# SGI-2022/Latent-Diffusion-Models-for-Shape-SDFs

Measured on AMD Instinct MI355X. Metric: SDF queries/sec on 256^3 grid (+ DDPM sample steps/sec), higher is better.
Workload: dtype bf16; 1 GPU; config4: decode B=64 shapes on a 256^3 grid on 1 rank (the whole grid is the one slab: no gather); batch=64, grid=256, latent_dim=256, decoder=DeepSDF 8x512 skip@4, parallelism=zslab1

## Files before the change

### latent-diffusion-models-for-shape-sdfs_amd/csrc/decoder_fs.hip

```cpp
#include "decoder_common.h"

namespace ldm {
namespace {
using namespace dec;

constexpr int kFsD = 4;

constexpr int kFsStep = 2048;
constexpr int kFsAct = 33 * 4 * 1024;
constexpr int kFsRed = 4 * 4 * 64 * 4;
constexpr int kFsWl = 512 * 4;
#ifndef FS_STAMP
#define FS_STAMP 0
#endif
constexpr int kFsStamp = FS_STAMP ? 128 * 8 : 0;
#ifndef FS_ABL
#define FS_ABL 0
#endif
static_assert(FS_ABL == 0 || FS_STAMP, "ablations are diagnostic builds");
constexpr int kFsLds = kFsAct + kFsRed + kFsWl + kFsStamp;
static_assert(kFsLds <= 160 * 1024, "LDS");

__host__ __device__ constexpr int fs_nparts(int S) { return S == 256 ? 15 : 16; }
__host__ __device__ constexpr int fs_nsteps(int S) { return S == 256 ? 384 : 448; }

template <typename T>
__global__ void fs_aux_pack_kernel(const float* __restrict__ beta, const float* __restrict__ wxyz,
                                   int B, T* __restrict__ aux) {
    const int id = blockIdx.x * blockDim.x + threadIdx.x;
    if (id >= B * 4 * 4 * 2 * 64) return;
    const int lane = id & 63;
    const int i = (id >> 6) & 1;
    const int slot = (id >> 7) & 3;
    const int w = (id >> 9) & 3;
    const int b = id >> 11;
    const int li = slot >> 1;
    const int p = slot & 1;
    float v[8] = {0, 0, 0, 0, 0, 0, 0, 0};
    if (lane < 32) {
        const int f = 128 * w + 64 * p + 32 * i + lane;
        const float* wx = wxyz + ((size_t)li * kHidden + f) * 3;
        const float bb = beta[((size_t)b * 2 + li) * kHidden + f];
        const float hi = Elem<T>::round(bb);
        v[0] = wx[0]; v[1] = wx[1]; v[2] = wx[2];
        v[3] = wx[0]; v[4] = wx[1]; v[5] = wx[2];
        v[6] = hi;    v[7] = bb - hi;
    }
    T* o = aux + (size_t)id * 8;
#pragma unroll
    for (int e = 0; e < 8; ++e) o[e] = (T)v[e];
}

struct FArgs {
    const uint8_t* stream;
    const uint8_t* aux;
    const float* w_last;
    const float* xyz;
    float* out;
    float b_last;
    int npts, tiles_per_shape, n_tiles;
    int N, k0;
    float vs, origin;
    const int32_t* bricks;
    const int32_t* count;
    int nb, nbt;
    GridDiv gd;
};

enum FsEpi { FE_NONE = 0, FE_LATE = 1, FE_EARLY = 2, FE_FIN0 = 3, FE_FIN1 = 4 };

struct FSrc {
    bool shape;
    uint32_t off;
    bool none = false;
};

struct FCtx {
    int lane, wave, h;
    uint32_t voff;
    char* smem;
    __amdgpu_buffer_rsrc_t rw;
    __amdgpu_buffer_rsrc_t ra;
    uint32_t s_beg, s_end;
    uint32_t s_iss;
    uint32_t baux_w;
    uint32_t aux_w;
    uint32_t aux_next;
    u32x4 auxn[2];
    u32x4 ring[kFsD][2];
    u32x4 b[4];
    float part[4];
    const f32x4* wlp;
    f32x4 wl[2][4];
    float* out;
    int npts, prev_shape, prev_local;
    float b_last;
    unsigned long long* st;
    int st_i;
    bool st_on;
    const int32_t* bricks;
    int N, nb, nbt;
};

__device__ __forceinline__ void stamp(FCtx& c) {
    if (FS_STAMP) {
        if (c.st_on && c.lane == 0 && c.st_i < 128) c.st[c.st_i] = __builtin_readcyclecounter();
        ++c.st_i;
    }
}

__device__ __forceinline__ u32x4 bld(__amdgpu_buffer_rsrc_t r, uint32_t voff, uint32_t soff) {
    return __builtin_bit_cast(u32x4, __builtin_amdgcn_raw_buffer_load_b128(r, voff, soff, 0));
}

__device__ __forceinline__ void load_aux(FCtx& c, FSrc s) {
    if (s.none) return;
    const __amdgpu_buffer_rsrc_t r = s.shape ? c.ra : c.rw;
    c.auxn[0] = bld(r, c.voff, s.off);
    c.auxn[1] = bld(r, c.voff + 1024u, s.off);
}

__device__ __forceinline__ uint32_t opaque(uint32_t v) {
    asm volatile("" : "+v"(v));
    return v;
}

__device__ __forceinline__ int opaque_s(int v) {
    asm volatile("" : "+s"(v));
    return v;
}

__device__ __forceinline__ char* lds_at(const FCtx& c, uint32_t off) {
    return c.smem + (opaque(c.voff) + off);
}
__device__ __forceinline__ char* lds_base(const FCtx& c, uint32_t off) {
    return c.smem + opaque(opaque(c.voff) + off);
}
__device__ __forceinline__ u32x4* act_wb(const FCtx& c, int late) {
    return reinterpret_cast<u32x4*>(lds_base(c, (uint32_t)(late + 4 * c.wave) * 4096u));
}
__device__ __forceinline__ u32x4* act_w(const FCtx& c, int late) {
    return reinterpret_cast<u32x4*>(lds_at(c, (uint32_t)(late + 4 * c.wave) * 4096u));
}
__device__ __forceinline__ const f32x4* wl_at(const FCtx& c, int p, int i) {
    const uint32_t h = opaque(c.voff) >> 9;
    return reinterpret_cast<const f32x4*>(
        c.smem + kFsAct + kFsRed + (((c.wave * 2 + p) * 2 + i) * 2) * 64 + h * 64);
}

__device__ __forceinline__ float* red_w(const FCtx& c) {
    return reinterpret_cast<float*>(c.smem + kFsAct + c.wave * 4 * 64 * 4 + (opaque(c.voff) >> 2));
}

__device__ __forceinline__ void fs_bar() {
    if (FS_ABL & 4) return;
    asm volatile("s_waitcnt lgkmcnt(0)\n\ts_barrier" ::: "memory");
}

__device__ __forceinline__ void read_b(FCtx& c, int pos) {
    const u32x4* p = reinterpret_cast<const u32x4*>(lds_at(c, pos * 4096));
#pragma unroll
    for (int n = 0; n < 4; ++n) c.b[n] = p[n * 64];
}

__device__ __forceinline__ void issue(FCtx& c, int r) {
    const uint32_t so = c.s_iss + (uint32_t)(r >> 1) * 2u * kFsStep;
    const uint32_t vo = c.voff + (uint32_t)(r & 1) * kFsStep;
    if (FS_ABL & 1) return;
    c.ring[r][0] = bld(c.rw, vo, so);
    c.ring[r][1] = bld(c.rw, vo + 1024u, so);
}

__device__ __forceinline__ uint32_t next_iss(const FCtx& c) {
    const uint32_t n = c.s_iss + 4u * kFsStep;
    return n == c.s_end ? c.s_beg : n;
}
__device__ __forceinline__ void next_group(FCtx& c) { c.s_iss = next_iss(c); }

__device__ __forceinline__ float relu_f(float x) {
    return __builtin_bit_cast(float, max(__builtin_bit_cast(int, x), 0));
}

__device__ __forceinline__ float acc_read(float a) {
    asm volatile("" : "+a"(a));
    return a;
}

__device__ __forceinline__ void fin1_unit(FCtx& c, const f32x16 (&accY)[2][4], int u) {
    const int t = u >> 1, s = u & 1;
    const int i = t >> 2, n = t & 3;
    const f32x4* w = wl_at(c, 1, i);
    float part = c.part[n];
#pragma unroll
    for (int q = 2 * s; q < 2 * s + 2; ++q) {
        const f32x4 wv = w[q];
#pragma unroll
        for (int e = 0; e < 4; ++e)
            part = fmaf(relu_f(acc_read(accY[i][n][4 * q + e])), wv[e], part);
    }
    c.part[n] = part;
}

template <typename T>
__device__ __forceinline__ void mfma_pair(f32x16 (&acc)[2][4], const u32x4& a0, const u32x4& a1,
                                          const u32x4& b, int n) {
    acc[0][n] = Elem<T>::mfma(a0, b, acc[0][n]);
    acc[1][n] = Elem<T>::mfma(a1, b, acc[1][n]);
}

template <typename T>
__device__ __forceinline__ void window_step(FCtx& c, f32x16 (&acc)[2][4],
                                            const f32x16 (&accY)[2][4], const u32x4& a0,
                                            const u32x4& a1, const u32x4* nb, int k, int r,
                                            u32x4* wbase) {
    uint32_t nxt = 0;
    if (k < 14) {
        const int t = k >> 1, s = k & 1;
        const int i = t >> 2, nn = t & 3;
        u32x4 f;
#pragma unroll
        for (int n = 0; n < 4; ++n) {
            unsigned w;
            if (r == 3 && n == 1) nxt = next_iss(c);
            const float e0 = accY[i][nn][8 * s + 2 * n], e1 = accY[i][nn][8 * s + 2 * n + 1];
            if (n < 3)
                Elem<T>::template pair_cvt1<false>(acc[0][n], acc[1][n], a0, a1, c.b[n], e0, e1,
                                                   w);
            else
                Elem<T>::template pair_cvt1<true>(acc[0][n], acc[1][n], a0, a1, c.b[n], e0, e1,
                                                  w);
            f[n] = w;
            c.b[n] = nb[n * 64];
            __builtin_amdgcn_sched_barrier(0);
        }
        issue(c, r);
        wbase[((2 * i + s) * 4 + nn) * 64] = f;
        if (r == 3) c.s_iss = nxt;
    } else {
        u32x4 f[2];
        const f32x16& y = accY[1][3];
#pragma unroll
        for (int p = 0; p < 4; ++p) {
            unsigned w0, w1;
            if (p < 3)
                Elem<T>::template pair_cvt2<false>(acc[0][p], acc[1][p], a0, a1, c.b[p], y[4 * p],
                                                   y[4 * p + 1], y[4 * p + 2], y[4 * p + 3], w0,
                                                   w1);
            else
                Elem<T>::template pair_cvt2<true>(acc[0][p], acc[1][p], a0, a1, c.b[p], y[4 * p],
                                                  y[4 * p + 1], y[4 * p + 2], y[4 * p + 3], w0,
                                                  w1);
            f[p >> 1][2 * (p & 1)] = w0;
            f[p >> 1][2 * (p & 1) + 1] = w1;
            c.b[p] = nb[p * 64];
            if (p == 1) wbase[(2 * 4 + 3) * 64] = f[0];
            __builtin_amdgcn_sched_barrier(0);
        }
        issue(c, r);
        wbase[(3 * 4 + 3) * 64] = f[1];
    }
    __builtin_amdgcn_sched_barrier(0);
}

template <typename T, int P>
__device__ __forceinline__ void window_step_fin(FCtx& c, f32x16 (&acc)[2][4],
                                                const f32x16 (&accY)[2][4], const u32x4& a0,
                                                const u32x4& a1, const u32x4* nb, int k, int r) {
    const int t = k >> 1, s = k & 1;
    const int i = t >> 2, nn = t & 3;
    const f32x16& y = accY[1][3];
    uint32_t nxt = 0;
    if (k == 0) {
        c.wlp = wl_at(c, P, 0);
#pragma unroll
        for (int q = 0; q < 4; ++q) c.wl[0][q] = c.wlp[q];
    }
#pragma unroll
    for (int n = 0; n < 4; ++n) {
        if (k < 14) {
            const int e = 8 * s + 2 * n;
            const float e0 = accY[i][nn][e], e1 = accY[i][nn][e + 1];
            const float w0 = c.wl[i][e >> 2][e & 3], w1 = c.wl[i][e >> 2][(e & 3) + 1];
            const int x = 2 * (k - 8) + n;
            if (k >= 8 && n < 2)
                Elem<T>::pair_fin3(acc[0][n], acc[1][n], a0, a1, c.b[n], e0, e1, w0, w1,
                                   c.part[nn], y[x], c.wl[1][x >> 2][x & 3], c.part[3]);
            else if (n < 3)
                Elem<T>::template pair_fin<false>(acc[0][n], acc[1][n], a0, a1, c.b[n], e0, e1,
                                                  w0, w1, c.part[nn]);
            else
                Elem<T>::template pair_fin<true>(acc[0][n], acc[1][n], a0, a1, c.b[n], e0, e1,
                                                 w0, w1, c.part[nn]);
        } else if (n < 2) {
            const int x = 12 + 2 * n;
            Elem<T>::template pair_fin<false>(acc[0][n], acc[1][n], a0, a1, c.b[n], y[x],
                                              y[x + 1], c.wl[1][3][x & 3],
                                              c.wl[1][3][(x & 3) + 1],
                                              c.part[3]);
        } else {
            mfma_pair<T>(acc, a0, a1, c.b[n], n);
        }
        if (r == 3 && n == 2) nxt = next_iss(c);
        c.b[n] = nb[n * 64];
        if (k == 6) c.wl[1][n] = c.wlp[8 + n];
        if (k == 14 && n == 2) {
            if (P == 0) {
#pragma unroll
                for (int m = 0; m < 4; ++m) asm volatile("" : "+v"(c.part[m]));
            } else {
                float* rw = red_w(c);
#pragma unroll
                for (int m = 0; m < 4; ++m) {
                    rw[m * 64] = c.part[m];
                    c.part[m] = 0.f;
                }
            }
        }
        __builtin_amdgcn_sched_barrier(0);
    }
    issue(c, r);
    if (r == 3) c.s_iss = nxt;
    __builtin_amdgcn_sched_barrier(0);
}

__device__ __forceinline__ void fin_store(const FCtx& c, int shape, int local) {
    const int lane = (int)(opaque(c.voff) >> 4);
    if (local < 0 || lane >= 32) return;
    const float* rr = reinterpret_cast<const float*>(
        c.smem + kFsAct + c.wave * 64 * 4 + (opaque(c.voff) >> 2));
    float s = 0.f;
#pragma unroll
    for (int w = 0; w < 4; ++w) s += rr[w * 4 * 64] + rr[w * 4 * 64 + 32];
    const int pt = local * kTilePoints + 32 * c.wave + lane;
    if (pt < c.npts) {
        const __amdgpu_buffer_rsrc_t ro = __builtin_amdgcn_make_buffer_rsrc(
            (void*)(c.out + (size_t)shape * c.npts), (short)0, 0x7ffffff0, 0x00020000);
        __builtin_amdgcn_raw_buffer_store_b32(__builtin_bit_cast(uint32_t, tanhf(s + c.b_last)),
                                              ro, (uint32_t)pt * 4u, 0, 2 );
    }
}

__device__ __forceinline__ int list_at(const int32_t* list, int i) {
    typedef const __attribute__((address_space(4))) int32_t* const_i32;
    return ((const_i32)(uintptr_t)list)[i];
}

__device__ __forceinline__ void brick_origin(int gid, int nb_, int& shape, int& i0, int& j0,
                                             int& k0) {
    const int nb = opaque_s(nb_);
    const int nb2 = nb * nb, nb3 = nb2 * nb;
    shape = gid / nb3;
    const int id = gid - shape * nb3;
    const int bz = id / nb2, r = id - bz * nb2;
    const int by = r / nb;
    i0 = 8 * (r - by * nb);
    j0 = 8 * by;
    k0 = 8 * bz;
}

__device__ __forceinline__ void fin_store_bricks(const FCtx& c, int tile) {
    const int lane = (int)(opaque(c.voff) >> 4);
    if (tile < 0 || lane >= 32) return;
    const float* rr = reinterpret_cast<const float*>(
        c.smem + kFsAct + c.wave * 64 * 4 + (opaque(c.voff) >> 2));
    float s = 0.f;
#pragma unroll
    for (int w = 0; w < 4; ++w) s += rr[w * 4 * 64] + rr[w * 4 * 64 + 32];
    const int gid = list_at(c.bricks, tile >> 2);
    LDM_DASSERT(gid >= 0 && gid < c.nbt);
    int shape, i0, j0, k0;
    brick_origin(gid, c.nb, shape, i0, j0, k0);
    const int idx = 128 * (tile & 3) + 32 * c.wave + lane;
    const int i = i0 + (idx & 7), j = j0 + ((idx >> 3) & 7);
    const int k = k0 + 2 * (tile & 3) + (c.wave >> 1);
    const int N = c.N;
    if ((unsigned)gid < (unsigned)c.nbt && i < N && j < N && k < N) {
        const __amdgpu_buffer_rsrc_t ro = __builtin_amdgcn_make_buffer_rsrc(
            (void*)(c.out + ((size_t)shape * N + k) * N * N), (short)0, 0x7ffffff0, 0x00020000);
        __builtin_amdgcn_raw_buffer_store_b32(__builtin_bit_cast(uint32_t, tanhf(s + c.b_last)),
                                              ro, (uint32_t)(j * N + i) * 4u, 0, 2 );
    }
}

template <int MODE>
__device__ __forceinline__ void fin_store_mode(const FCtx& c) {
    if (MODE == kModeBricks) fin_store_bricks(c, c.prev_local);
    else fin_store(c, c.prev_shape, c.prev_local);
}

template <typename T, int EK, int K0, int BAR, bool WIN = false>
__device__ __forceinline__ void group4(FCtx& c, f32x16 (&acc)[2][4], const f32x16 (&accY)[2][4],
                                       int p0, const char* gb = nullptr, u32x4* wb = nullptr,
                                       uint32_t* go = nullptr) {
    static_assert(WIN || EK == FE_NONE, "windows run through steps16e");
    constexpr int BP = 1;
    const bool carry = go != nullptr;
    const char* gbase = WIN ? gb : carry ? c.smem + *go + 4096 : lds_base(c, (p0 + 1) * 4096);
#pragma unroll
    for (int r = 0; r < 4; ++r) {
        const bool last = carry && r == 3;
        uint32_t nxt = 0;
        if (last) {
            nxt = next_iss(c);
            *go = opaque(*go + 4u * 4096u);
        }
        const u32x4* nb =
            reinterpret_cast<const u32x4*>(last ? c.smem + *go : gbase + r * 4096);
        const u32x4 a0 = c.ring[r][0], a1 = c.ring[r][1];
        const int k = K0 + r;
        if (r == BAR) {
#pragma unroll
            for (int n = 0; n < BP; ++n) mfma_pair<T>(acc, a0, a1, c.b[n], n);
            for (int n = 0; n < BP; ++n) {
                __builtin_amdgcn_sched_group_barrier(0x008, 2, 0);
            }
            __builtin_amdgcn_sched_barrier(0);
            fs_bar();
            __builtin_amdgcn_sched_barrier(0);
#pragma unroll
            for (int n = 0; n < BP; ++n) c.b[n] = nb[n * 64];
#pragma unroll
            for (int n = BP; n < 4; ++n) {
                mfma_pair<T>(acc, a0, a1, c.b[n], n);
                c.b[n] = nb[n * 64];
            }
            issue(c, r);
            for (int n = 0; n < BP; ++n) __builtin_amdgcn_sched_group_barrier(0x100, 1, 0);
            for (int n = BP; n < 4; ++n) {
                __builtin_amdgcn_sched_group_barrier(0x008, 2, 0);
                __builtin_amdgcn_sched_group_barrier(0x100, 1, 0);
            }
        } else if ((EK == FE_LATE || EK == FE_EARLY) && k < 15 && !(FS_ABL & 2)) {
            window_step<T>(c, acc, accY, a0, a1, nb, k, r, wb);
            if (r == 3) return;
            continue;
        } else if ((EK == FE_FIN0 || EK == FE_FIN1) && k < 15 && !(FS_ABL & 2)) {
            window_step_fin<T, EK == FE_FIN1>(c, acc, accY, a0, a1, nb, k, r);
            if (r == 3) return;
            continue;
        } else {
#pragma unroll
            for (int n = 0; n < 4; ++n) {
                mfma_pair<T>(acc, a0, a1, c.b[n], n);
                c.b[n] = nb[n * 64];
            }
            issue(c, r);
            if (last) c.s_iss = nxt;
#pragma unroll
            for (int n = 0; n < 4; ++n) {
                __builtin_amdgcn_sched_group_barrier(0x008, 2, 0);
                if (last && n == 0) {
                    __builtin_amdgcn_sched_group_barrier(0x004, 3, 0);
                    __builtin_amdgcn_sched_group_barrier(0x002, 1, 0);
                }
                __builtin_amdgcn_sched_group_barrier(0x100, 1, 0);
            }
        }
        __builtin_amdgcn_sched_group_barrier(0x020, 2, 0);
        __builtin_amdgcn_sched_barrier(0);
    }
    if (!carry) next_group(c);
}

template <typename T, int EK, bool BAR>
__device__ __forceinline__ void steps16e(FCtx& c, f32x16 (&acc)[2][4],
                                         const f32x16 (&accY)[2][4], int p0) {
    const char* gb = lds_base(c, (p0 + 1) * 4096);
    u32x4* wb = EK == FE_LATE ? act_wb(c, 16) : EK == FE_EARLY ? act_wb(c, 0) : nullptr;
    group4<T, EK, 0, -1, true>(c, acc, accY, p0, gb, wb);
    group4<T, EK, 4, -1, true>(c, acc, accY, p0 + 4, gb + 4 * 4096, wb);
    group4<T, EK, 8, -1, true>(c, acc, accY, p0 + 8, gb + 8 * 4096, wb);
    group4<T, EK, 12, BAR ? 3 : -1, true>(c, acc, accY, p0 + 12, gb + 12 * 4096, wb);
}

template <typename T>
__device__ __forceinline__ void steps_plain(FCtx& c, f32x16 (&acc)[2][4],
                                            const f32x16 (&accY)[2][4], int pos0, int j0, int j1) {
    if (j0 >= j1) return;
    uint32_t go = opaque(opaque(c.voff) + (uint32_t)(pos0 + j0) * 4096u);
#pragma unroll 1
    for (int j = j0; j < j1; j += 4)
        group4<T, FE_NONE, 0, -1>(c, acc, accY, pos0 + j, nullptr, nullptr, &go);
}

template <typename T, int EK, bool E16, int MODE = kModeGrid>
__device__ __forceinline__ void run_part(FCtx& c, f32x16 (&acc)[2][4], const f32x16 (&accY)[2][4],
                                         int nk, bool mid, bool endbar, FSrc naux, int pos0,
                                         bool bar0) {
    const f32x16 zero = {};
    const u32x4 a0 = c.auxn[0], a1 = c.auxn[1];
    if (bar0) {
#pragma unroll
        for (int n = 0; n < 4; ++n) {
            acc[0][n] = Elem<T>::mfma(a0, c.b[n], zero);
            acc[1][n] = Elem<T>::mfma(a1, c.b[n], zero);
        }
        load_aux(c, naux);
        fs_bar();
        read_b(c, pos0);
    } else {
        const u32x4* p = reinterpret_cast<const u32x4*>(lds_at(c, pos0 * 4096));
#pragma unroll
        for (int n = 0; n < 4; ++n) {
            acc[0][n] = Elem<T>::mfma(a0, c.b[n], zero);
            acc[1][n] = Elem<T>::mfma(a1, c.b[n], zero);
            c.b[n] = p[n * 64];
        }
        load_aux(c, naux);
#pragma unroll
        for (int n = 0; n < 4; ++n) {
            __builtin_amdgcn_sched_group_barrier(0x008, 2, 0);
            __builtin_amdgcn_sched_group_barrier(0x100, 1, 0);
        }
        __builtin_amdgcn_sched_group_barrier(0x020, 2, 0);
        __builtin_amdgcn_sched_barrier(0);
    }
    if (EK == FE_NONE) {
#pragma unroll
        for (int i = 0; i < 2; ++i)
#pragma unroll
            for (int n = 0; n < 4; ++n) asm volatile("" ::"a"(accY[i][n]));
    }
    stamp(c);
    if (!E16 && EK != FE_NONE) {
        if (mid || (endbar && nk == 16)) steps16e<T, EK, true>(c, acc, accY, pos0);
        else steps16e<T, EK, false>(c, acc, accY, pos0);
        if (EK == FE_FIN1) {
            stamp(c);
            fin_store_mode<MODE>(c);
        }
        stamp(c);
        if (endbar && nk == 32) {
            steps_plain<T>(c, acc, accY, pos0, 16, 28);
            group4<T, FE_NONE, 0, 3>(c, acc, accY, pos0 + 28);
        } else {
            steps_plain<T>(c, acc, accY, pos0, 16, nk);
        }
    } else if (E16) {
        static_assert(!E16 || EK == FE_EARLY, "E16 parts convert part 0 of their own layer");
        steps_plain<T>(c, acc, accY, pos0, 0, 12);
        group4<T, FE_NONE, 0, 3>(c, acc, accY, pos0 + 12);
        stamp(c);
        if (endbar) steps16e<T, EK, true>(c, acc, accY, pos0 + 16);
        else steps16e<T, EK, false>(c, acc, accY, pos0 + 16);
    } else {
        steps_plain<T>(c, acc, accY, pos0, 0, nk < 16 ? nk : 16);
        stamp(c);
        steps_plain<T>(c, acc, accY, pos0, 16, nk);
    }
    stamp(c);
}

template <typename T>
__device__ __forceinline__ void acc_to_lds(FCtx& c, const f32x16 (&acc)[2][4]) {
    u32x4* p = act_w(c, 16);
#pragma unroll
    for (int i = 0; i < 2; ++i)
#pragma unroll
        for (int n = 0; n < 4; ++n) {
            u32x4 f0, f1;
            acc_to_frags<T>(acc[i][n], f0, f1);
            p[(2 * i * 4 + n) * 64] = f0;
            p[((2 * i + 1) * 4 + n) * 64] = f1;
        }
}

template <typename T, bool LATE>
__device__ __forceinline__ void layer0_part(FCtx& c, FSrc naux) {
    const u32x4 a[2] = {c.auxn[0], c.auxn[1]};
    u32x4* p = act_w(c, LATE ? 16 : 0);
    f32x16 t[2];
    t[0] = Elem<T>::mfma_v(a[0], c.b[0]);
#pragma unroll
    for (int q = 0; q < 8; ++q) {
        const int i = q & 1, n = q >> 1;
        if (q < 7) t[(q + 1) & 1] = Elem<T>::mfma_v(a[(q + 1) & 1], c.b[(q + 1) >> 1]);
        if (q == 0) {
            asm volatile("s_nop 10" : "+v"(t[0]));
            load_aux(c, naux);
            stamp(c);
        }
        __builtin_amdgcn_sched_barrier(0);
        u32x4 f0, f1;
        acc_to_frags<T>(t[q & 1], f0, f1);
        p[(2 * i * 4 + n) * 64] = f0;
        p[((2 * i + 1) * 4 + n) * 64] = f1;
        __builtin_amdgcn_sched_barrier(0);
    }
    stamp(c);
}

template <typename T, int S, int MODE>
__global__ __launch_bounds__(256, 1) void dec_fs_kernel(FArgs a) {
    __shared__ __attribute__((aligned(16))) char smem[kFsLds];
    FCtx c;
    c.lane = threadIdx.x & 63;
    c.wave = __builtin_amdgcn_readfirstlane(threadIdx.x >> 6);
    c.h = c.lane >> 5;
    c.voff = (uint32_t)c.lane * 16u;
    c.smem = smem;
    c.out = a.out;
    c.npts = a.npts;
    c.b_last = a.b_last;
    c.prev_shape = 0;
    c.prev_local = -1;
    c.st = reinterpret_cast<unsigned long long*>(smem + kFsAct + kFsRed + kFsWl);
    c.st_i = 0;
    c.st_on = false;
    float* wl = reinterpret_cast<float*>(smem + kFsAct + kFsRed);

    for (int i = threadIdx.x; i < 512; i += 256) wl[i] = a.w_last[i];
    __syncthreads();
    const int n_tiles = MODE == kModeBricks ? 4 * min(max(a.count[0], 0), a.nbt) : a.n_tiles;
    if (MODE == kModeBricks) {
        c.bricks = a.bricks;
        c.N = a.N;
        c.nb = a.nb;
        c.nbt = a.nbt;
    }
    if ((int)blockIdx.x >= n_tiles) return;

    constexpr int NST = fs_nsteps(S);
    constexpr int NP = fs_nparts(S);
    constexpr uint32_t kFlags = 0x00020000u;
    c.rw = __builtin_amdgcn_make_buffer_rsrc((void*)a.stream, (short)0, 0x7ffffff0, kFlags);
    c.ra = __builtin_amdgcn_make_buffer_rsrc((void*)a.aux, (short)0, 0x7ffffff0, kFlags);
    c.s_beg = (uint32_t)c.wave * NST * kFsStep;
    c.s_end = c.s_beg + NST * kFsStep;
    c.s_iss = c.s_beg;
    c.baux_w = (uint32_t)(4 * NST + c.wave * NP) * kFsStep;
    auto brick_of = [&](int tile) -> int {
        return min(max(list_at(a.bricks, tile >> 2), 0), a.nbt - 1);
    };
    auto shape_aux = [&](int tile) -> uint32_t {
        if (MODE == kModeBricks) {
            const int nb = opaque_s(a.nb);
            return ((uint32_t)(brick_of(tile) / (nb * nb * nb)) * 4u + (uint32_t)c.wave) * 4u *
                   kFsStep;
        }
        return ((uint32_t)(tile / a.tiles_per_shape) * 4u + (uint32_t)c.wave) * 4u * kFsStep;
    };
    auto bias = [&](int pi) -> FSrc { return FSrc{false, c.baux_w + (uint32_t)pi * kFsStep}; };
    auto shp = [&](int slot) -> FSrc { return FSrc{true, c.aux_w + (uint32_t)slot * kFsStep}; };
    c.aux_w = shape_aux(blockIdx.x);
#pragma unroll
    for (int r = 0; r < kFsD; ++r) issue(c, r);
    next_group(c);

    f32x16 accA[2][4], accB[2][4];
#pragma unroll
    for (int i = 0; i < 2; ++i)
#pragma unroll
        for (int n = 0; n < 4; ++n) accB[i][n] = f32x16{};
#pragma unroll
    for (int n = 0; n < 4; ++n) c.part[n] = 0.f;
#pragma unroll 1
    for (int tile = blockIdx.x; tile < n_tiles; tile += gridDim.x) {
        int shape, local, bi0 = 0, bj0 = 0, bk0 = 0;
        if (MODE == kModeBricks) {
            brick_origin(brick_of(tile), a.nb, shape, bi0, bj0, bk0);
            local = tile;
        } else {
            shape = tile / a.tiles_per_shape;
            local = tile - shape * a.tiles_per_shape;
        }
        {
            const int nt = tile + (int)gridDim.x;
            c.aux_next = nt < n_tiles ? shape_aux(nt) : c.aux_w;
        }
        c.st_on = FS_STAMP && c.wave == 0 && tile == (int)blockIdx.x + (int)gridDim.x;
        c.st_i = 0;
        stamp(c);
        load_aux(c, shp(0));
        const uint32_t lv = opaque(c.voff);
        const bool hi = lv >= 512u;
        const uint32_t p0 = (uint32_t)local * kTilePoints;
        uint32_t ti = 0, tj = 0, tk = 0;
        if (MODE == kModeGrid) {
            grid_first(p0, (uint32_t)a.N, a.gd, ti, tj, tk);
            tk += (uint32_t)a.k0;
        }
        const float* row = nullptr;
        if (MODE == kModePoints) {
            row = a.xyz + (size_t)shape * a.npts * 3;
            asm volatile("" : "+s"(row));
        }
#pragma unroll
        for (int n = 0; n < 4; ++n) {
            int pt = local * kTilePoints + 32 * n + (int)((lv >> 4) & 31u);
            if (pt >= a.npts) pt = a.npts - 1;
            float x, y, z;
            if (MODE == kModeBricks) {
                const int idx = 128 * (tile & 3) + 32 * n + (int)((lv >> 4) & 31u);
                const int m = a.N - 1;
                x = grid_axis(min(bi0 + (idx & 7), m), a.vs, a.origin);
                y = grid_axis(min(bj0 + ((idx >> 3) & 7), m), a.vs, a.origin);
                z = grid_axis(min(bk0 + (idx >> 6), m), a.vs, a.origin);
            } else if (MODE == kModePoints) {
                const float* qq = row + (size_t)pt * 3;
                x = qq[0];
                y = qq[1];
                z = qq[2];
            } else {
                const uint32_t off =
                    grid_tail_off(p0, 32u * n + ((lv >> 4) & 31u), (uint32_t)a.npts);
                uint32_t vi, vj, vk;
                grid_voxel(ti, tj, tk, off, (uint32_t)a.N, a.gd.m, vi, vj, vk);
                x = grid_axis((int)vi, a.vs, a.origin);
                y = grid_axis((int)vj, a.vs, a.origin);
                z = grid_axis((int)vk, a.vs, a.origin);
            }
            const float xh = Elem<T>::round(x), yh = Elem<T>::round(y), zh = Elem<T>::round(z);
            u32x4 f;
            f[0] = hi ? 0u : Elem<T>::pack(xh, yh);
            f[1] = hi ? 0u : Elem<T>::pack(zh, x - xh);
            f[2] = hi ? 0u : Elem<T>::pack(y - yh, z - zh);
            f[3] = hi ? 0u : Elem<T>::pack(1.f, 1.f);
            reinterpret_cast<u32x4*>(lds_at(c, 32u * 4096u))[n * 64] = f;
        }
        read_b(c, 32);

        layer0_part<T, false>(c, shp(1));
        layer0_part<T, true>(c, bias(2));

        int pi = 2;
        run_part<T, FE_FIN1, false, MODE>(c, accA, accB, 32, true, false, bias(pi + 1), 0, true);
        run_part<T, FE_EARLY, true>(c, accB, accA, 32, true, true, bias(pi + 2), 0, false);
        pi += 2;
        constexpr int L2P = S == 256 ? 3 : 4;
#pragma unroll 1
        for (int l = 2; l < L2P; ++l, pi += 2) {
            const FSrc nx = (S == 512 && l == 3) ? shp(2) : bias(pi + 2);
            run_part<T, FE_LATE, false>(c, accA, accB, 32, true, false, bias(pi + 1), 0,
                                                false);
            run_part<T, FE_EARLY, true>(c, accB, accA, 32, true, true, nx, 0, false);
        }
        if (S == 256) {
            run_part<T, FE_LATE, false>(c, accA, accB, 32, true, false, shp(2), 0,
                                                false);
            fs_bar();
            acc_to_lds<T>(c, accA);
            stamp(c);
            run_part<T, FE_NONE, false>(c, accA, accB, 16, false, false, shp(3), 16, true);
            run_part<T, FE_EARLY, false>(c, accB, accA, 16, false, true, bias(pi + 3),
                                                  16, false);
            pi += 3;
        } else {
            run_part<T, FE_LATE, false>(c, accA, accB, 32, true, false, shp(3), 0,
                                                false);
            run_part<T, FE_EARLY, true>(c, accB, accA, 32, true, true, bias(pi + 2), 0,
                                                 false);
            pi += 2;
        }
#pragma unroll 1
        for (int l = 5; l < 7; ++l, pi += 2) {
            run_part<T, FE_LATE, false>(c, accA, accB, 32, true, false, bias(pi + 1), 0,
                                                 false);
            run_part<T, FE_EARLY, true>(c, accB, accA, 32, true, true, bias(pi + 2), 0,
                                                 false);
        }
        run_part<T, FE_LATE, false>(c, accA, accB, 32, true, false, bias(pi + 1), 0,
                                             false);
        run_part<T, FE_FIN0, false>(c, accB, accA, 32, false, true, FSrc{true, 0, true},
                                             0, false);
        c.prev_shape = shape;
        c.prev_local = local;
        c.aux_w = c.aux_next;
    }
#pragma unroll
    for (int u = 0; u < 16; ++u) fin1_unit(c, accB, u);
    {
        float* rw = red_w(c);
#pragma unroll
        for (int n = 0; n < 4; ++n) rw[n * 64] = c.part[n];
    }
    fs_bar();
    fin_store_mode<MODE>(c);
    asm volatile("s_waitcnt vmcnt(0)" ::: "memory");
    if (FS_STAMP && c.wave == 0) {
        __builtin_amdgcn_s_waitcnt(0);
        for (int k = c.lane; k < 128; k += 64)
            reinterpret_cast<unsigned long long*>(a.out)[(size_t)blockIdx.x * 128 + k] = c.st[k];
    }
}

template <typename T, int S>
void launch_fs(const FArgs& a, bool points, hipStream_t s, int grid) {
    if (points)
        hipLaunchKernelGGL((dec_fs_kernel<T, S, kModePoints>), dim3(grid), dim3(256), 0, s, a);
    else
        hipLaunchKernelGGL((dec_fs_kernel<T, S, kModeGrid>), dim3(grid), dim3(256), 0, s, a);
}

template <typename T, int S>
void launch_fs_bricks(const FArgs& a, hipStream_t s, int grid) {
    hipLaunchKernelGGL((dec_fs_kernel<T, S, kModeBricks>), dim3(grid), dim3(256), 0, s, a);
}

}

size_t decoder_fs_aux_bytes(int B) { return (size_t)B * 4 * 4 * kFsStep; }

int decoder_fs_n_stages(int skip_width) { return fs_nsteps(skip_width == 253 ? 256 : 512); }

int decoder_fs_fwd(const ldm_decoder_t* w, const float* beta, const float* xyz, int B, int npts,
                   int N, int k0, float vs, float origin, float* out, void* ws, size_t ws_bytes,
                   hipStream_t s, int num_cus, const int32_t* bricks, const int32_t* count,
                   int n_bricks) {
    const int S = w->skip_width == 253 ? 256 : 512;
    LDM_REQUIRE(w->n_stages == fs_nsteps(S), LDM_EINVAL, "split layout: n_stages %d != %d",
                w->n_stages, fs_nsteps(S));
    LDM_REQUIRE(ws != nullptr && ws_bytes >= decoder_fs_aux_bytes(B) && LDM_ALIGNED(ws, 16),
                LDM_ENOSPC, "workspace too small: need %zu bytes, got %zu",
                decoder_fs_aux_bytes(B), ws_bytes);
    LDM_REQUIRE((size_t)B * 4 * 4 * kFsStep < 0x7ffffff0u, LDM_EINVAL,
                "split layout: %d shapes exceed the aux buffer range", B);
    {
        const int n = B * 4 * 4 * 2 * 64;
        if (w->dtype == LDM_BF16)
            hipLaunchKernelGGL(fs_aux_pack_kernel<__bf16>, dim3((n + 255) / 256), dim3(256), 0, s,
                               beta, w->wxyz, B, (__bf16*)ws);
        else
            hipLaunchKernelGGL(fs_aux_pack_kernel<_Float16>, dim3((n + 255) / 256), dim3(256), 0,
                               s, beta, w->wxyz, B, (_Float16*)ws);
        if (int e = launch_status("fs_aux_pack")) return e;
    }
    FArgs a;
    a.stream = (const uint8_t*)w->weights;
    a.aux = (const uint8_t*)ws;
    a.w_last = w->w_last;
    a.xyz = xyz;
    a.out = out;
    a.b_last = w->b_last;
    a.npts = npts;
    a.tiles_per_shape = (npts + kTilePoints - 1) / kTilePoints;
    a.n_tiles = B * a.tiles_per_shape;
    a.bricks = bricks;
    a.count = count;
    a.nb = (N + 7) / 8;
    a.nbt = n_bricks;
    const int mode = bricks ? kModeBricks : xyz ? kModePoints : kModeGrid;
    if (mode == kModeBricks) a.n_tiles = 4 * n_bricks;
    a.N = N;
    a.k0 = k0;
    a.vs = vs;
    a.origin = origin;
    a.gd = mode == kModeGrid ? grid_div(N) : GridDiv{0, 0, 0};
    const int grid = a.n_tiles < num_cus ? a.n_tiles : num_cus;
    if (mode != kModeBricks) {
        const bool points = mode == kModePoints;
        if (w->dtype == LDM_BF16) {
            if (S == 256) launch_fs<__bf16, 256>(a, points, s, grid);
            else launch_fs<__bf16, 512>(a, points, s, grid);
        } else {
            if (S == 256) launch_fs<_Float16, 256>(a, points, s, grid);
            else launch_fs<_Float16, 512>(a, points, s, grid);
        }
    } else if (w->dtype == LDM_BF16) {
        if (S == 256) launch_fs_bricks<__bf16, 256>(a, s, grid);
        else launch_fs_bricks<__bf16, 512>(a, s, grid);
    } else {
        if (S == 256) launch_fs_bricks<_Float16, 256>(a, s, grid);
        else launch_fs_bricks<_Float16, 512>(a, s, grid);
    }
    return launch_status("ldm_decoder_fwd(split)");
}

}
```

### latent-diffusion-models-for-shape-sdfs_amd/csrc/grid_index.h

```cpp
#pragma once
#include <stdint.h>

#if defined(__HIPCC__) || defined(__CUDACC__)
#define LDM_HD __host__ __device__ inline __attribute__((always_inline))
#else
#define LDM_HD inline
#endif

namespace ldm {
namespace dec {

struct GridDiv {
    uint32_t m, mw, sh;
};

inline GridDiv grid_div(int N) {
    GridDiv d;
    d.m = (uint32_t)(((1ull << 32) + (uint32_t)N - 1) / (uint32_t)N);
    uint32_t lg = 0;
    while ((1u << lg) < (uint32_t)N) ++lg;
    d.sh = 31 + lg;
    d.mw = (uint32_t)(((1ull << d.sh) + (uint32_t)N - 1) / (uint32_t)N);
    return d;
}

LDM_HD uint32_t grid_mulhi(uint32_t a, uint32_t b) {
    return (uint32_t)(((uint64_t)a * b) >> 32);
}

LDM_HD uint32_t grid_mul24(uint32_t a, uint32_t b) {
    return (a & 0xffffffu) * (b & 0xffffffu);
}

LDM_HD void grid_first(uint32_t p0, uint32_t N, GridDiv d, uint32_t& i, uint32_t& j,
                       uint32_t& k) {
    const uint32_t row = (uint32_t)(((uint64_t)p0 * d.mw) >> d.sh);
    i = p0 - row * N;
    k = grid_mulhi(row, d.m);
    j = row - k * N;
}

LDM_HD void grid_voxel(uint32_t i0, uint32_t j0, uint32_t k0, uint32_t off, uint32_t N,
                       uint32_t m, uint32_t& i, uint32_t& j, uint32_t& k) {
    const uint32_t x = i0 + off;
    const uint32_t cx = grid_mulhi(x, m);
    i = x - grid_mul24(cx, N);
    const uint32_t y = j0 + cx;
    const uint32_t cy = grid_mulhi(y, m);
    j = y - grid_mul24(cy, N);
    k = k0 + cy;
}

LDM_HD uint32_t grid_tail_off(uint32_t p0, uint32_t want, uint32_t npts) {
    const uint32_t last = npts - 1u - p0;
    return want < last ? want : last;
}

}
}
```

Baseline: 487.3 million queries/s.

## Interleave final tanh store into next layer's MFMA steps and simplify grid-row coordinates

Moves the final-layer reduction, tanh and output store of the previous tile out of its own serialized epilogue and splits it into pieces scheduled between the MFMAs of the next part, using explicit sched_group_barrier orderings. Replaces tanhf with a custom branch-free tanh split into stages so each stage can ride in an MFMA slot. When N is a multiple of 128, tiles lie within one grid row, so per-point coordinate decoding uses a simple row form instead of the div/mod voxel walk. The aim is to hide epilogue latency and cut scalar/vector overhead, at the cost of tanh accuracy differences and tight hand scheduling that could spill or mis-order.

```diff
diff --git a/latent-diffusion-models-for-shape-sdfs_amd/csrc/decoder_fs.hip b/latent-diffusion-models-for-shape-sdfs_amd/csrc/decoder_fs.hip
--- a/latent-diffusion-models-for-shape-sdfs_amd/csrc/decoder_fs.hip
+++ b/latent-diffusion-models-for-shape-sdfs_amd/csrc/decoder_fs.hip
@@ -1,4 +1,5 @@
 #include "decoder_common.h"
+#include "tanh_select.h"
 
 namespace ldm {
 namespace {
@@ -65,6 +66,7 @@
     const int32_t* count;
     int nb, nbt;
     GridDiv gd;
+    int row;
 };
 
 enum FsEpi { FE_NONE = 0, FE_LATE = 1, FE_EARLY = 2, FE_FIN0 = 3, FE_FIN1 = 4 };
@@ -335,9 +337,92 @@
     if (pt < c.npts) {
         const __amdgpu_buffer_rsrc_t ro = __builtin_amdgcn_make_buffer_rsrc(
             (void*)(c.out + (size_t)shape * c.npts), (short)0, 0x7ffffff0, 0x00020000);
-        __builtin_amdgcn_raw_buffer_store_b32(__builtin_bit_cast(uint32_t, tanhf(s + c.b_last)),
-                                              ro, (uint32_t)pt * 4u, 0, 2 );
-    }
+        __builtin_amdgcn_raw_buffer_store_b32(
+            __builtin_bit_cast(uint32_t, tanh_select(s + c.b_last)), ro, (uint32_t)pt * 4u, 0,
+            2 );
+    }
+}
+
+struct FinSt {
+    const float* rr;
+    float v[8];
+    float s;
+    uint32_t lv, pt, off;
+    __amdgpu_buffer_rsrc_t ro;
+    TanhSel t;
+};
+
+__device__ __forceinline__ void fin_piece(const FCtx& c, FinSt& f, int u) {
+    switch (u) {
+    case 0:
+        f.rr = reinterpret_cast<const float*>(c.smem + kFsAct + c.wave * 64 * 4 +
+                                              ((opaque(c.voff) & 0x1ffu) >> 2));
+        break;
+    case 1:
+#pragma unroll
+        for (int w = 0; w < 2; ++w) {
+            f.v[2 * w] = f.rr[w * 4 * 64];
+            f.v[2 * w + 1] = f.rr[w * 4 * 64 + 32];
+        }
+        f.lv = opaque(c.voff);
+        break;
+    case 2:
+#pragma unroll
+        for (int w = 2; w < 4; ++w) {
+            f.v[2 * w] = f.rr[w * 4 * 64];
+            f.v[2 * w + 1] = f.rr[w * 4 * 64 + 32];
+        }
+        f.pt = (uint32_t)(c.prev_local * kTilePoints + 32 * c.wave) + (f.lv >> 4);
+        break;
+    case 3:
+        f.off = f.lv < 512u && f.pt < (uint32_t)c.npts ? f.pt * 4u : 0x80000000u;
+        break;
+    case 4:
+        f.s = 0.f;
+        f.s += f.v[0] + f.v[1];
+        f.s += f.v[2] + f.v[3];
+        break;
+    case 5:
+        f.s += f.v[4] + f.v[5];
+        f.s += f.v[6] + f.v[7];
+        f.t.x = f.s + c.b_last;
+        break;
+    case 6:
+        tanh_sel_head(f.t);
+        tanh_sel_tail(f.t);
+        break;
+    case 7:
+        tanh_sel_exp2(f.t);
+        break;
+    case 8:
+        tanh_sel_scale(f.t);
+        asm volatile("" : "+v"(f.t.v));
+        break;
+    case 9:
+        tanh_sel_poly(f.t);
+        break;
+    case 10:
+        tanh_sel_rcp(f.t);
+        f.ro = __builtin_amdgcn_make_buffer_rsrc((void*)(c.out + (size_t)c.prev_shape * c.npts),
+                                                 (short)0, 0x7ffffff0, 0x00020000);
+        break;
+    default:
+        __builtin_amdgcn_raw_buffer_store_b32(__builtin_bit_cast(uint32_t, tanh_sel_end(f.t)),
+                                              f.ro, f.off, 0, 2 );
+    }
+}
+
+template <int V1, int S1, int V2, int S2>
+__device__ __forceinline__ void fin_order() {
+    __builtin_amdgcn_sched_group_barrier(0x008, 1, 0);
+    __builtin_amdgcn_sched_group_barrier(0x002, V1, 0);
+    __builtin_amdgcn_sched_group_barrier(0x004, S1, 0);
+    __builtin_amdgcn_sched_group_barrier(0x008, 1, 0);
+    __builtin_amdgcn_sched_group_barrier(0x100, 3, 0);
+    __builtin_amdgcn_sched_group_barrier(0x400, 1, 0);
+    __builtin_amdgcn_sched_group_barrier(0x002, V2, 0);
+    __builtin_amdgcn_sched_group_barrier(0x004, S2, 0);
+    __builtin_amdgcn_sched_group_barrier(0x040, 1, 0);
 }
 
 __device__ __forceinline__ int list_at(const int32_t* list, int i) {
@@ -388,11 +473,13 @@
     else fin_store(c, c.prev_shape, c.prev_local);
 }
 
-template <typename T, int EK, int K0, int BAR, bool WIN = false>
+template <typename T, int EK, int K0, int BAR, bool WIN = false, bool FIN = false>
 __device__ __forceinline__ void group4(FCtx& c, f32x16 (&acc)[2][4], const f32x16 (&accY)[2][4],
                                        int p0, const char* gb = nullptr, u32x4* wb = nullptr,
                                        uint32_t* go = nullptr) {
     static_assert(WIN || EK == FE_NONE, "windows run through steps16e");
+    static_assert(!FIN || (BAR == 3 && !WIN), "the store rides in the three plain compiled steps");
+    FinSt fin;
     constexpr int BP = 1;
     const bool carry = go != nullptr;
     const char* gbase = WIN ? gb : carry ? c.smem + *go + 4096 : lds_base(c, (p0 + 1) * 4096);
@@ -438,6 +525,25 @@
             window_step_fin<T, EK == FE_FIN1>(c, acc, accY, a0, a1, nb, k, r);
             if (r == 3) return;
             continue;
+        } else if (FIN) {
+#pragma unroll
+            for (int n = 0; n < 4; ++n) {
+                fin_piece(c, fin, 4 * r + n);
+                mfma_pair<T>(acc, a0, a1, c.b[n], n);
+                c.b[n] = nb[n * 64];
+                if (n == 3) issue(c, r);
+                switch (4 * r + n) {
+                case 0: fin_order<2, 0, 3, 0>(); break;
+                case 2: fin_order<4, 2, 1, 0>(); break;
+                case 4: fin_order<2, 0, 3, 0>(); break;
+                case 5: fin_order<4, 0, 3, 0>(); break;
+                case 8: fin_order<4, 0, 2, 0>(); break;
+                case 10: fin_order<2, 3, 0, 3>(); break;
+                case 11: fin_order<5, 0, 0, 1>(); break;
+                default: fin_order<5, 1, 3, 1>();
+                }
+                if (n < 3) __builtin_amdgcn_sched_barrier(0);
+            }
         } else {
 #pragma unroll
             for (int n = 0; n < 4; ++n) {
@@ -483,7 +589,7 @@
         group4<T, FE_NONE, 0, -1>(c, acc, accY, pos0 + j, nullptr, nullptr, &go);
 }
 
-template <typename T, int EK, bool E16, int MODE = kModeGrid>
+template <typename T, int EK, bool E16, int MODE = kModeGrid, bool FIN = false>
 __device__ __forceinline__ void run_part(FCtx& c, f32x16 (&acc)[2][4], const f32x16 (&accY)[2][4],
                                          int nk, bool mid, bool endbar, FSrc naux, int pos0,
                                          bool bar0) {
@@ -527,7 +633,7 @@
         else steps16e<T, EK, false>(c, acc, accY, pos0);
         if (EK == FE_FIN1) {
             stamp(c);
-            fin_store_mode<MODE>(c);
+            if (MODE == kModeBricks) fin_store_mode<MODE>(c);
         }
         stamp(c);
         if (endbar && nk == 32) {
@@ -539,7 +645,7 @@
     } else if (E16) {
         static_assert(!E16 || EK == FE_EARLY, "E16 parts convert part 0 of their own layer");
         steps_plain<T>(c, acc, accY, pos0, 0, 12);
-        group4<T, FE_NONE, 0, 3>(c, acc, accY, pos0 + 12);
+        group4<T, FE_NONE, 0, 3, false, FIN>(c, acc, accY, pos0 + 12);
         stamp(c);
         if (endbar) steps16e<T, EK, true>(c, acc, accY, pos0 + 16);
         else steps16e<T, EK, false>(c, acc, accY, pos0 + 16);
@@ -685,38 +791,59 @@
             row = a.xyz + (size_t)shape * a.npts * 3;
             asm volatile("" : "+s"(row));
         }
-#pragma unroll
-        for (int n = 0; n < 4; ++n) {
-            int pt = local * kTilePoints + 32 * n + (int)((lv >> 4) & 31u);
-            if (pt >= a.npts) pt = a.npts - 1;
-            float x, y, z;
-            if (MODE == kModeBricks) {
-                const int idx = 128 * (tile & 3) + 32 * n + (int)((lv >> 4) & 31u);
-                const int m = a.N - 1;
-                x = grid_axis(min(bi0 + (idx & 7), m), a.vs, a.origin);
-                y = grid_axis(min(bj0 + ((idx >> 3) & 7), m), a.vs, a.origin);
-                z = grid_axis(min(bk0 + (idx >> 6), m), a.vs, a.origin);
-            } else if (MODE == kModePoints) {
-                const float* qq = row + (size_t)pt * 3;
-                x = qq[0];
-                y = qq[1];
-                z = qq[2];
-            } else {
-                const uint32_t off =
-                    grid_tail_off(p0, 32u * n + ((lv >> 4) & 31u), (uint32_t)a.npts);
+        if (MODE == kModeGrid && a.row) {
+            const float y = grid_axis((int)tj, a.vs, a.origin);
+            const float z = grid_axis((int)tk, a.vs, a.origin);
+            const float yh = Elem<T>::round(y), zh = Elem<T>::round(z);
+            const uint32_t f2 = hi ? 0u : Elem<T>::pack(y - yh, z - zh);
+            const uint32_t f3 = hi ? 0u : Elem<T>::pack(1.f, 1.f);
+#pragma unroll
+            for (int n = 0; n < 4; ++n) {
                 uint32_t vi, vj, vk;
-                grid_voxel(ti, tj, tk, off, (uint32_t)a.N, a.gd.m, vi, vj, vk);
-                x = grid_axis((int)vi, a.vs, a.origin);
-                y = grid_axis((int)vj, a.vs, a.origin);
-                z = grid_axis((int)vk, a.vs, a.origin);
+                grid_voxel_row(ti, tj, tk, 32u * n + ((lv >> 4) & 31u), vi, vj, vk);
+                const float x = grid_axis((int)vi, a.vs, a.origin);
+                const float xh = Elem<T>::round(x);
+                u32x4 f;
+                f[0] = hi ? 0u : Elem<T>::pack(xh, yh);
+                f[1] = hi ? 0u : Elem<T>::pack(zh, x - xh);
+                f[2] = f2;
+                f[3] = f3;
+                reinterpret_cast<u32x4*>(lds_at(c, 32u * 4096u))[n * 64] = f;
             }
-            const float xh = Elem<T>::round(x), yh = Elem<T>::round(y), zh = Elem<T>::round(z);
-            u32x4 f;
-            f[0] = hi ? 0u : Elem<T>::pack(xh, yh);
-            f[1] = hi ? 0u : Elem<T>::pack(zh, x - xh);
-            f[2] = hi ? 0u : Elem<T>::pack(y - yh, z - zh);
-            f[3] = hi ? 0u : Elem<T>::pack(1.f, 1.f);
-            reinterpret_cast<u32x4*>(lds_at(c, 32u * 4096u))[n * 64] = f;
+        } else {
+#pragma unroll
+            for (int n = 0; n < 4; ++n) {
+                int pt = local * kTilePoints + 32 * n + (int)((lv >> 4) & 31u);
+                if (pt >= a.npts) pt = a.npts - 1;
+                float x, y, z;
+                if (MODE == kModeBricks) {
+                    const int idx = 128 * (tile & 3) + 32 * n + (int)((lv >> 4) & 31u);
+                    const int m = a.N - 1;
+                    x = grid_axis(min(bi0 + (idx & 7), m), a.vs, a.origin);
+                    y = grid_axis(min(bj0 + ((idx >> 3) & 7), m), a.vs, a.origin);
+                    z = grid_axis(min(bk0 + (idx >> 6), m), a.vs, a.origin);
+                } else if (MODE == kModePoints) {
+                    const float* qq = row + (size_t)pt * 3;
+                    x = qq[0];
+                    y = qq[1];
+                    z = qq[2];
+                } else {
+                    const uint32_t off =
+                        grid_tail_off(p0, 32u * n + ((lv >> 4) & 31u), (uint32_t)a.npts);
+                    uint32_t vi, vj, vk;
+                    grid_voxel(ti, tj, tk, off, (uint32_t)a.N, a.gd.m, vi, vj, vk);
+                    x = grid_axis((int)vi, a.vs, a.origin);
+                    y = grid_axis((int)vj, a.vs, a.origin);
+                    z = grid_axis((int)vk, a.vs, a.origin);
+                }
+                const float xh = Elem<T>::round(x), yh = Elem<T>::round(y), zh = Elem<T>::round(z);
+                u32x4 f;
+                f[0] = hi ? 0u : Elem<T>::pack(xh, yh);
+                f[1] = hi ? 0u : Elem<T>::pack(zh, x - xh);
+                f[2] = hi ? 0u : Elem<T>::pack(y - yh, z - zh);
+                f[3] = hi ? 0u : Elem<T>::pack(1.f, 1.f);
+                reinterpret_cast<u32x4*>(lds_at(c, 32u * 4096u))[n * 64] = f;
+            }
         }
         read_b(c, 32);
 
@@ -725,7 +852,8 @@
 
         int pi = 2;
         run_part<T, FE_FIN1, false, MODE>(c, accA, accB, 32, true, false, bias(pi + 1), 0, true);
-        run_part<T, FE_EARLY, true>(c, accB, accA, 32, true, true, bias(pi + 2), 0, false);
+        run_part<T, FE_EARLY, true, MODE, MODE != kModeBricks>(c, accB, accA, 32, true, true,
+                                                               bias(pi + 2), 0, false);
         pi += 2;
         constexpr int L2P = S == 256 ? 3 : 4;
 #pragma unroll 1
@@ -846,6 +974,7 @@
     a.vs = vs;
     a.origin = origin;
     a.gd = mode == kModeGrid ? grid_div(N) : GridDiv{0, 0, 0};
+    a.row = mode == kModeGrid && grid_row_tiles(N);
     const int grid = a.n_tiles < num_cus ? a.n_tiles : num_cus;
     if (mode != kModeBricks) {
         const bool points = mode == kModePoints;
diff --git a/latent-diffusion-models-for-shape-sdfs_amd/csrc/grid_index.h b/latent-diffusion-models-for-shape-sdfs_amd/csrc/grid_index.h
--- a/latent-diffusion-models-for-shape-sdfs_amd/csrc/grid_index.h
+++ b/latent-diffusion-models-for-shape-sdfs_amd/csrc/grid_index.h
@@ -51,6 +51,15 @@
     k = k0 + cy;
 }
 
+inline bool grid_row_tiles(int N) { return N % 128 == 0; }
+
+LDM_HD void grid_voxel_row(uint32_t i0, uint32_t j0, uint32_t k0, uint32_t off, uint32_t& i,
+                           uint32_t& j, uint32_t& k) {
+    i = i0 + off;
+    j = j0;
+    k = k0;
+}
+
 LDM_HD uint32_t grid_tail_off(uint32_t p0, uint32_t want, uint32_t npts) {
     const uint32_t last = npts - 1u - p0;
     return want < last ? want : last;
diff --git a/latent-diffusion-models-for-shape-sdfs_amd/csrc/tanh_select.h b/latent-diffusion-models-for-shape-sdfs_amd/csrc/tanh_select.h
--- /dev/null
+++ b/latent-diffusion-models-for-shape-sdfs_amd/csrc/tanh_select.h
@@ -0,0 +1,67 @@
+#pragma once
+
+namespace ldm {
+namespace dec {
+
+struct TanhSel {
+    float x;
+    float t;
+    float ph, pl;
+    float n;
+    float v;
+    float lo;
+    float r;
+};
+
+__device__ __forceinline__ void tanh_sel_head(TanhSel& s) {
+#pragma clang fp contract(off)
+    s.t = __builtin_fabsf(s.x) * 2.0f;
+    s.ph = s.t * 0x1.715476p+0f;
+}
+__device__ __forceinline__ void tanh_sel_tail(TanhSel& s) {
+    s.pl = __builtin_fmaf(s.t, 0x1.715476p+0f, -s.ph);
+    s.pl = __builtin_fmaf(s.t, 0x1.4ae0bep-26f, s.pl);
+    s.n = __builtin_rintf(s.ph);
+}
+__device__ __forceinline__ void tanh_sel_exp2(TanhSel& s) {
+#pragma clang fp contract(off)
+    const float a = (s.ph - s.n) + s.pl;
+    s.v = __builtin_amdgcn_exp2f(a);
+}
+__device__ __forceinline__ void tanh_sel_scale(TanhSel& s) {
+    float v = __builtin_amdgcn_ldexpf(s.v, (int)s.n);
+    v = s.t < -0x1.9d1dap+6f ? 0.0f : v;
+    s.v = s.t > 0x1.62e430p+6f ? __builtin_inff() : v;
+}
+__device__ __forceinline__ void tanh_sel_poly(TanhSel& s) {
+#pragma clang fp contract(off)
+    const float y = __builtin_fabsf(s.x);
+    const float x2 = s.x * s.x;
+    float p = __builtin_fmaf(x2, -0x1.758e7ap-8f, 0x1.521192p-6f);
+    p = __builtin_fmaf(x2, p, -0x1.b8389cp-5f);
+    p = __builtin_fmaf(x2, p, 0x1.110704p-3f);
+    p = __builtin_fmaf(x2, p, -0x1.555532p-2f);
+    s.lo = __builtin_fmaf(x2, y * p, y);
+}
+__device__ __forceinline__ void tanh_sel_rcp(TanhSel& s) {
+    s.r = __builtin_amdgcn_rcpf(s.v + 1.0f);
+}
+__device__ __forceinline__ float tanh_sel_end(const TanhSel& s) {
+    const float hi = __builtin_fmaf(s.r, -2.0f, 1.0f);
+    return __builtin_copysignf(__builtin_fabsf(s.x) < 0.625f ? s.lo : hi, s.x);
+}
+
+__device__ __forceinline__ float tanh_select(float x) {
+    TanhSel s;
+    s.x = x;
+    tanh_sel_head(s);
+    tanh_sel_tail(s);
+    tanh_sel_exp2(s);
+    tanh_sel_scale(s);
+    tanh_sel_poly(s);
+    tanh_sel_rcp(s);
+    return tanh_sel_end(s);
+}
+
+}
+}
```

After: 488.8 million queries/s, median of 6. About the same (+0.3%).
